# gallilmaimon/DISSC

Hardware: AMD Instinct MI355X
Metric: audio-sec/sec (RTF) HiFi-GAN resynth, 10s x32 batch (higher is better)
Workload: dtype f32

## Files before the change

dissc_amd/csrc/common.h:

```cpp
#pragma once
#include <hip/hip_runtime.h>
#include <stdint.h>
#include <stdio.h>

#include <atomic>
#include <mutex>
#include <string>
#include <vector>

#include "../../include/dissc_hip.h"

#ifndef DISSC_EXPERIMENTAL
#define DISSC_EXPERIMENTAL 0
#endif

namespace dissc {

void set_error(const char* fmt, ...);

#define DISSC_OPTION_LIST_DEFAULT(X) \
  X(multistream, 1, "multistream") \
  X(pair_dma, 1, "pair_dma") \
  X(precision, 0, "precision") \
  X(enc_precision, 0, "enc_precision") \
  X(use_mfma32, 1, "mfma32") \
  X(ragged_enum, 1, "ragged_enum") \
  X(lin128, 1, "lin128") \
  X(conv2s128, 1, "conv2s128") \
  X(xcd_order, 11, "xcd_order") \
  X(xcd_mg, 0, "xcd_mg") \
  X(small_grid, 1, "small_grid") \
  X(kernel_dbg, 0, "kernel_dbg") \
  X(wino_sv, 1, "wino_sv") \
  X(wino8_c64_wide, 3, "wino8_c64_wide") \
  X(wino8_mask, 0450770550, "wino8_mask") \
  X(wino8_r4_mask, 0770770010, "wino8_r4_mask") \
  X(wino8_r4, 1, "wino8_r4") \
  X(wino8, 1, "wino8") \
  X(wino, 1, "wino") \
  X(hubert_split, 1, "hubert_split") \
  X(pair_max_c, 32, "pair_max_c") \
  X(pair_f23, 3, "pair_f23") \
  X(pair_tc6, 3, "pair_tc6") \
  X(pair_f23_c64, 1, "pair_f23_c64")
#define DISSC_OPTION_LIST_EXPERIMENTAL(X) \
  X(graphs, 0, "graphs") \
  X(graph_frames, 2048, "graph_frames") \
  X(enc_tc, 0, "enc_tc") \
  X(s2tc_xmode, 0, "s2tc_xmode") \
  X(pair_wino, 0, "pair_wino") \
  X(pairw_chv, 2, "pairw_chv")
#if DISSC_EXPERIMENTAL
#define DISSC_OPTION_LIST(X) DISSC_OPTION_LIST_DEFAULT(X) DISSC_OPTION_LIST_EXPERIMENTAL(X)
#else
#define DISSC_OPTION_LIST(X) DISSC_OPTION_LIST_DEFAULT(X)
#endif
struct Options {
#define DISSC_OPT_FIELD(f, d, k) int f = d;
  DISSC_OPTION_LIST(DISSC_OPT_FIELD)
#undef DISSC_OPT_FIELD
#if !DISSC_EXPERIMENTAL
#define DISSC_OPT_CONST(f, d, k) static constexpr int f = d;
  DISSC_OPTION_LIST_EXPERIMENTAL(DISSC_OPT_CONST)
#undef DISSC_OPT_CONST
#endif
  int cfg_for_bm[5] = {6, 5, 7, 1, 0};
  int cfg32_for_bm[4] = {3, 2, 1, 0};
};
extern Options g_defaults;
extern thread_local const Options* t_opts;
inline const Options& opts() { return t_opts ? *t_opts : g_defaults; }
struct OptScope {
  const Options* prev;
  explicit OptScope(const Options* o) : prev(t_opts) { t_opts = o; }
  ~OptScope() { t_opts = prev; }
  OptScope(const OptScope&) = delete;
  OptScope& operator=(const OptScope&) = delete;
};

#define DISSC_HIP_CHECK(expr)                                                       \
  do {                                                                              \
    hipError_t _e = (expr);                                                         \
    if (_e != hipSuccess) {                                                         \
      dissc::set_error("%s failed: %s (%s:%d)", #expr, hipGetErrorString(_e),       \
                       __FILE__, __LINE__);                                         \
      return DISSC_EHIP;                                                            \
    }                                                                               \
  } while (0)

typedef float f32x4 __attribute__((ext_vector_type(4)));

struct DeviceOnce {
  std::mutex mu;
  std::atomic<bool> done[64];
  DeviceOnce() {
    for (auto& d : done) d.store(false, std::memory_order_relaxed);
  }
// ... 262 lines not shown
```

dissc_amd/csrc/generator.hip:

```cpp
#include <stdarg.h>
#include <stdlib.h>
#include <string.h>

#include <atomic>
#include <exception>
#include <functional>
#include <map>
#include <mutex>
#include <string>
#include <thread>
#include <tuple>
#include <vector>

#include <algorithm>

#include "common.h"

namespace dissc {

static thread_local char g_err[512] = "";
void set_error(const char* fmt, ...) {
  va_list ap;
  va_start(ap, fmt);
  vsnprintf(g_err, sizeof(g_err), fmt, ap);
// ... 2 lines not shown

Options g_defaults;
thread_local const Options* t_opts = nullptr;

}

using namespace dissc;

[[maybe_unused]] static int g_graph_hits = 0, g_graph_captures = 0;

enum class ChainForm : uint8_t {
  pairs,
  bf3_block,
  bf3_pairs,
};
enum class PairForm : uint8_t {
  direct,
  direct_dma,
  td,
  fused,
  fused_td,
};
enum class ConvForm : uint8_t { direct, f43, f63, f54 };
struct PairPlan {
  PairForm form = PairForm::direct;
  ConvForm conv[2] = {ConvForm::direct, ConvForm::direct};
  uint8_t reg_form = 0;
};
struct ChainPlan {
  ChainForm form = ChainForm::pairs;
  PairPlan pair[3];
};

constexpr int WINO_MIN_C = 64;
constexpr int WINO_C64_KMIN = 3;
static bool wino_wanted(int C, int KS) {
  if (!opts().wino || C < WINO_MIN_C) return false;
  if (C < 128 && KS < WINO_C64_KMIN) return false;
  return wino_supported(C, C, KS, 1);
}

static int w8_shape_bit(int C, int KS, int dil) {
  const int cls = C >= 256 ? 2 : C >= 128 ? 1 : 0;
  return 9 * cls + 3 * (KS == 11 ? 2 : KS == 7 ? 1 : 0) + (dil == 1 ? 0 : dil == 3 ? 1 : 2);
}
static ConvForm td_conv_form(int C, int KS, int dil) {
  if (!opts().wino8 || !wino8_supported(C, C, KS, dil) || !((opts().wino8_mask >> w8_shape_bit(C, KS, dil)) & 1))
    return ConvForm::f43;
  const bool r4 = opts().wino8_r4 && wino8_r4_supported(C, KS, dil) && ((opts().wino8_r4_mask >> w8_shape_bit(C, KS, dil)) & 1);
  return r4 ? ConvForm::f54 : ConvForm::f63;
}

static int pair_reg_form(int C, int KS, int dil) {
  if (C == 64) return KS == 3 && opts().pair_f23 != 0 && opts().pair_f23_c64 && pair_f23_supported(C, KS, dil) ? 1 : 0;
  if (C != 16 && C != 32) return 0;
  const int stage = C == 32 ? 1 : 2;
  if (KS == 3) return pair_f23_supported(C, KS, dil) && (opts().pair_f23 & (stage << 2)) ? 1 : 0;
  if (!(opts().pair_f23 & stage)) return 0;
  const int tc6_bit = (C == 32 ? 1 : 4) << (KS == 11 ? 1 : 0);
  if ((KS == 7 || KS == 11) && (opts().pair_tc6 & tc6_bit) && pair_tc6_supported(C, KS, dil)) return 2;
  return pair_f23_supported(C, KS, dil) ? 1 : 0;
}
static bool pairw_wanted(int C, int KS, int dil) {
  if (pair_reg_form(C, KS, dil)) return true;
  if (!opts().pair_wino || !pairw_supported(C, KS, dil)) return false;
  if (opts().pair_wino >= 2) return true;
  if (C == 32) return KS == 11 && dil <= 3;
  return C == 64 && KS == 3 && dil == 1;
}

static ChainPlan plan_chain(int C, int KS, const int* dil, int prec) {
  ChainPlan cp;
  if (prec == 1 && resblock_bf3_supported(C, KS, dil)) {
    cp.form = C >= 64 ? ChainForm::bf3_pairs : ChainForm::bf3_block;
    return cp;
  }
  bool fused = prec == 0 && (C < 32 || opts().use_mfma32) && C <= opts().pair_max_c;
  for (int m = 0; m < 3; ++m) fused = fused && respair_supported(C, KS, dil[m]);
  bool all_td = prec == 0 && opts().wino && C > 32 && wino_wanted(C, KS);
  for (int m = 0; m < 3; ++m) all_td = all_td && wino_supported(C, C, KS, dil[m]) && pairw_wanted(C, KS, dil[m]);
  for (int m = 0; m < 3; ++m) {
    PairPlan& p = cp.pair[m];
    const int d = dil[m];
    const bool td = prec == 0 && wino_wanted(C, KS) && wino_supported(C, C, KS, d);
    const bool fuse_td = prec == 0 && opts().wino && pairw_wanted(C, KS, d) && (C > 32 ? td : C <= opts().pair_max_c) &&
                         (fused || all_td || m == 0);
    if (fuse_td) {
      p.form = PairForm::fused_td;
      p.reg_form = (uint8_t)pair_reg_form(C, KS, d);
    } else if (fused) {
      p.form = PairForm::fused;
    } else if (td) {
      p.form = PairForm::td;
      p.conv[0] = td_conv_form(C, KS, d);
      p.conv[1] = td_conv_form(C, KS, 1);
    } else if (opts().pair_dma && prec == 0 && opts().use_mfma32 && C >= 32 && C % KC == 0) {
      p.form = PairForm::direct_dma;
    }
  }
  return cp;
}

static double pair_macs(const PairPlan& p, int C, int KS, bool executed) {
  const double direct = (double)C * C * KS;
  auto conv = [&](ConvForm f) {
    return f == ConvForm::f43 ? wino_executed_macs_per_t(C, KS)
         : f == ConvForm::f63 ? wino8_executed_macs_per_t(C, KS, 3)
// ... 567 lines not shown
  launch_conv_post(ACC, g->post_w, g->post_b, lengths, mul, B, ch, g->post_KS, Tmax * mul, ld,
                   (long long)ch * ld, 0.01f, wav_out, Tmax * mul, stream);
  DISSC_HIP_CHECK(hipGetLastError());
  return DISSC_OK;
}

int dissc_wav_postprocess(float* wav, const int32_t* n_samples, int B, int ld, void* stream) {
  if (!wav || !n_samples || B <= 0) {
    set_error("dissc_wav_postprocess: bad argument");
    return DISSC_EINVAL;
  }
  launch_wav_postprocess(wav, n_samples, B, ld, (hipStream_t)stream);
  DISSC_HIP_CHECK(hipGetLastError());
  return DISSC_OK;
}

static int conv_once(DevConv& dc, const float* x, float* y, const int32_t* lengths, int B,
                     int ldx, int ldo, int Lmax, float in_slope, hipStream_t stream) {
  int rc = run_conv(dc, x, y, nullptr, nullptr, lengths, Lmax, 1, B, dc.CIN, ldx, ldo, Lmax,
                    in_slope, EPI_STORE, 1.f, stream);
  hipError_t e = hipStreamSynchronize(stream);
  free_conv(dc);
  if (rc) return rc;
  DISSC_HIP_CHECK(e);
  return DISSC_OK;
}

int dissc_conv1d(const float* x, const float* w_host, const float* bias_host, float* y,
                 const int32_t* lengths, int B, int Cin, int Cout, int k, int dilation, int ldx,
                 int ldo, int Lmax, float in_slope, void* stream) {
  if (!x || !w_host || !y || k % 2 != 1 || dilation < 1) {
    set_error("dissc_conv1d: bad argument");
    return DISSC_EINVAL;
  }
  DevConv dc;
  int rc;
  if (opts().wino8 >= 2 && wino8_supported(Cout, Cin, k, dilation))
    rc = make_wino8(w_host, bias_host, Cout, k, dilation, dc, opts().wino8_r4 >= 2 && wino8_r4_supported(Cout, k, dilation) ? 4 : 3);
  else if (opts().wino >= 2 && wino_supported(Cout, Cin, k, dilation))
    rc = make_wino(w_host, bias_host, Cout, k, dilation, dc);
  else
    rc = make_conv(w_host, bias_host, Cout, Cin, k, dilation, dc);
  if (rc) return rc;
  return conv_once(dc, x, y, lengths, B, ldx, ldo, Lmax, in_slope, (hipStream_t)stream);
}

static int pair_run(int mode, const DevConv& c1, const DevConv& c2, const DevPairW& pw, const float* x, float* tmp, float* y,
                    float* acc, const int32_t* lengths, int B, int C, int ld, int Lmax, float slope, int epi, float mrf_div,
                    hipStream_t st) {
  int rc;
  switch (mode) {
    case 0:
    case 2:
      if ((rc = run_conv(c1, x, tmp, nullptr, nullptr, lengths, Lmax, 1, B, C, ld, ld, Lmax, slope, EPI_STORE, 1.f, st))) return rc;
      return run_conv(c2, tmp, y, x, acc, lengths, Lmax, 1, B, C, ld, ld, Lmax, slope, epi, mrf_div, st);
    case 1:
      return launch_respair(c1, c2, x, y, acc, lengths, Lmax, 1, B, Lmax, ld, slope, epi, mrf_div, st);
    case 3:
      return launch_respair_wino(pw, x, y, acc, lengths, Lmax, 1, B, Lmax, ld, slope, epi, mrf_div, st);
    default:
      set_error("pair mode %d", mode);
      return DISSC_EINVAL;
  }
}

static int pair_make(int mode, const float* w1, const float* b1, const float* w2, const float* b2, int C, int k, int d,
                     DevConv& c1, DevConv& c2, DevPairW& pw) {
  int rc;
  if (mode == 2) {
    if (!wino_supported(C, C, k, d) && !(C == 32 && (k == 3 || k == 7 || k == 11) && (d == 1 || d == 3 || d == 5))) {
      set_error("pair mode 2: no conv_wino instance for C = %d, k = %d, d = %d", C, k, d);
      return DISSC_EINVAL;
    }
    if ((rc = make_wino(w1, b1, C, k, d, c1))) return rc;
    return make_wino(w2, b2, C, k, 1, c2);
  }
  if (mode == 3) return make_pairw(w1, b1, w2, b2, C, k, d, pair_reg_form(C, k, d), pw);
  if ((rc = make_conv(w1, b1, C, C, k, d, c1))) return rc;
  return make_conv(w2, b2, C, C, k, 1, c2);
}

int dissc_respair1d(const float* x, const float* w1_host, const float* b1_host, const float* w2_host, const float* b2_host,
                    float* y, float* acc, const int32_t* lengths, int B, int C, int k, int dilation, int ld, int Lmax,
                    float slope, int epi, float mrf_div, int mode, void* stream) {
  if (!x || !w1_host || !w2_host || !y || k % 2 != 1 || dilation < 1 || B <= 0 || epi < EPI_RES || epi > EPI_MRF_DIV ||
      (epi != EPI_RES && !acc)) {
    set_error("dissc_respair1d: bad argument");
    return DISSC_EINVAL;
  }
  DevConv c1, c2;
  DevPairW pw;
  float* tmp = nullptr;
  int rc = pair_make(mode, w1_host, b1_host, w2_host, b2_host, C, k, dilation, c1, c2, pw);
  if (!rc && (mode == 0 || mode == 2) && hipMalloc((void**)&tmp, (size_t)B * C * ld * sizeof(float)) != hipSuccess) {
    set_error("dissc_respair1d: hipMalloc");
    rc = DISSC_ENOMEM;
  }
  if (!rc) rc = pair_run(mode, c1, c2, pw, x, tmp, y, acc, lengths, B, C, ld, Lmax, slope, epi, mrf_div, (hipStream_t)stream);
  const hipError_t e = hipStreamSynchronize((hipStream_t)stream);
  if (tmp) (void)hipFree(tmp);
  free_conv(c1);
  free_conv(c2);
  free_pairw(pw);
  if (rc) return rc;
  DISSC_HIP_CHECK(e);
  return DISSC_OK;
}

int dissc_pair_info(int C, int k, int dilation, int* form_out, int* tile_out) {
  const int form = pair_reg_form(C, k, dilation);
  if (!pair_form_supported(form, C, k, dilation)) {
    set_error("dissc_pair_info: no instance for C = %d, k = %d, dilation %d", C, k, dilation);
    return DISSC_EINVAL;
  }
  if (form_out) *form_out = form;
  if (tile_out) *tile_out = pair_reg_tile(form, C, k, dilation);
  return DISSC_OK;
}

int dissc_conv_info(int Cin, int Cout, int k, int dilation, int up, int B, int Lmax_out, DisscConvLaunch* out, int max_out,
                    int* n_out) {
  if (Cin < 1 || Cout < 1 || k < 1 || dilation < 1 || up < 1 || B < 1 || Lmax_out < 1 || max_out < 0 || (max_out && !out) ||
      (up == 1 && k % 2 != 1) || (up > 1 && ((k - up) % 2 != 0 || k < up || dilation != 1))) {
    set_error("dissc_conv_info: bad argument");
    return DISSC_EINVAL;
  }
  std::vector<ConvTGroup> plan;
  if (up > 1) convT_groups(Cout, k, up, plan);
  else plan.push_back(ConvTGroup{0, 1, 0, k});
  int n = 0;
  for (const ConvTGroup& g : plan) {
    DevConv dc;
    conv_geometry(dc, Cout * g.np, Cin, g.ntap, up > 1 ? 1 : dilation, 1, 1, up > 1 ? -g.dlo : -1);
    int family, cfg, bm, bn;
    const int rc = conv_launch_info(dc, B, Lmax_out, &family, &cfg, &bm, &bn);
    if (rc) return rc;
    if (n < max_out) {
      DisscConvLaunch& o = out[n];
      o.family = family; o.cfg = cfg; o.bm = bm; o.bn = bn; o.rows = dc.M;
      o.p0 = g.p0; o.np = g.np; o.ntap = g.ntap;
      o.pad_left = dc.pad_left >= 0 ? dc.pad_left : ((dc.KS - 1) * dc.dil) / 2;
    }
    ++n;
  }
  if (n_out) *n_out = n;
  return DISSC_OK;
}
// ... 187 lines not shown
```

dissc_amd/csrc/pair_host.hip:

```cpp
#include <string.h>

#include <algorithm>
#include <vector>

#include "common.h"
#include "respair_f23.h"

namespace dissc {

bool pair_f23_supported(int C, int KS, int dil) {
  if (!(dil == 1 || dil == 3 || dil == 5)) return false;
  if (C == 64) return KS == 3;
  return (C == 16 || C == 32) && (KS == 11 || (KS == 3 && DISSC_EXPERIMENTAL));
}
bool pair_tc6_supported(int C, int KS, int dil) { return C == 32 && (KS == 7 || KS == 11) && (dil == 1 || dil == 3 || dil == 5); }
bool pairw_supported(int C, int KS, int dil) {
  if (!pairw43_built()) return false;
  if (!(dil == 1 || dil == 3 || dil == 5)) return false;
  if (C == 32) return KS == 7 || KS == 11;
  if (C == 64) return KS == 3;
  return false;
}
bool pair_form_supported(int form, int C, int KS, int dil) {
  return form == 2 ? pair_tc6_supported(C, KS, dil) : form == 1 ? pair_f23_supported(C, KS, dil) : pairw_supported(C, KS, dil);
}

static const double kF23G[4][3] = {{1.0, 0.0, 0.0}, {0.5, 0.5, 0.5}, {0.5, -0.5, 0.5}, {0.0, 0.0, 1.0}};
static const double kTc6G[6][4] = {{1.0 / 4, 0.0, 0.0, 0.0},
                                   {-1.0 / 6, -1.0 / 6, -1.0 / 6, -1.0 / 6},
                                   {-1.0 / 6, 1.0 / 6, -1.0 / 6, 1.0 / 6},
                                   {1.0 / 24, 2.0 / 24, 4.0 / 24, 8.0 / 24},
                                   {1.0 / 24, -2.0 / 24, 4.0 / 24, -8.0 / 24},
                                   {0.0, 0.0, 0.0, 1.0}};

static std::vector<float> transform_taps(const float* w, int C, int KS, const double* G, int points, int taps) {
  const int NS = (KS + taps - 1) / taps;
  std::vector<float> U((size_t)points * C * C * NS);
  size_t o = 0;
  for (int p = 0; p < points; ++p)
    for (int cc = 0; cc < C * C; ++cc)
      for (int j = 0; j < NS; ++j) {
        double u = 0.0;
        for (int i = 0; i < taps; ++i)
          if (j + NS * i < KS) u += G[p * taps + i] * (double)w[(size_t)cc * KS + j + NS * i];
        U[o++] = (float)u;
      }
  return U;
}

static int pack_pair_reg(const float* w, float** dev, int C, int KS, int form) {
  if ((form != 1 && form != 2) || (C != 16 && C != 32 && C != 64) || (form == 2 && C != 32) || (C == 64 && KS != 3)) {
    set_error("pack_pair_reg: no layout for form %d, C = %d", form, C);
    return DISSC_EINVAL;
  }
  const int points = form == 2 ? 6 : 4, taps = form == 2 ? 4 : 3, NS = (KS + taps - 1) / taps;
  const std::vector<float> U = transform_taps(w, C, KS, form == 2 ? &kTc6G[0][0] : &kF23G[0][0], points, taps);
  auto u = [&](int p, int co, int ci, int j) { return U[(((size_t)p * C + co) * C + ci) * NS + j]; };
  std::vector<float> packed(U.size());
  size_t o = 0;
  if (C == 16) {
    for (int j = 0; j < NS; ++j)
      for (int p = 0; p < 4; ++p)
        for (int lane = 0; lane < 64; ++lane)
          for (int cq = 0; cq < 4; ++cq) packed[o++] = u(p, lane & 15, 4 * cq + (lane >> 4), j);
  } else if (C == 64) {
    for (int st = 0; st < 8; ++st)
      for (int p = 0; p < 4; ++p)
        for (int mi = 0; mi < 2; ++mi)
          for (int lane = 0; lane < 64; ++lane)
            for (int e = 0; e < 4; ++e) packed[o++] = u(p, 32 * mi + (lane & 31), 8 * st + 2 * e + (lane >> 5), 0);
  } else if (form == 1) {
    for (int c = 0; c < 2; ++c)
      for (int j = 0; j < NS; ++j)
        for (int p = 0; p < 4; ++p)
          for (int hf = 0; hf < 2; ++hf)
            for (int lane = 0; lane < 64; ++lane)
              for (int e = 0; e < 4; ++e) packed[o++] = u(p, lane & 31, 16 * c + 2 * (4 * hf + e) + (lane >> 5), j);
  } else {
    for (int c = 0; c < 2; ++c)
      for (int j = 0; j < NS; ++j)
        for (int hf = 0; hf < 2; ++hf)
          for (int p = 0; p < 6; ++p)
            for (int lane = 0; lane < 64; ++lane)
              for (int e = 0; e < 4; ++e) packed[o++] = u(p, lane & 31, 16 * c + 2 * (4 * hf + e) + (lane >> 5), j);
  }
  return upload(packed, dev);
}

int make_pairw(const float* w1, const float* b1, const float* w2, const float* b2, int C, int KS, int dil, int form, DevPairW& pw) {
  pw.form = form;
  if (!pair_form_supported(form, C, KS, dil)) {
    set_error("make_pairw: no instance for C = %d, k = %d, dilation %d", C, KS, dil);
    return DISSC_EINVAL;
  }
  pw.C = C; pw.KS = KS; pw.dil = dil;
  auto pack = [&](const float* w, float** dev) {
    return form ? pack_pair_reg(w, dev, C, KS, form) : pack_pairw43(w, C, KS, dev);
  };
  int rc = pack(w1, &pw.w1);
  if (!rc) rc = pack(w2, &pw.w2);
  std::vector<float> bb(C, 0.f);
  if (b1) memcpy(bb.data(), b1, C * sizeof(float));
  if (!rc) rc = upload(bb, &pw.b1);
  std::fill(bb.begin(), bb.end(), 0.f);
  if (b2) memcpy(bb.data(), b2, C * sizeof(float));
  if (!rc) rc = upload(bb, &pw.b2);
  return rc;
}

void free_pairw(DevPairW& pw) {
  for (float** q : {&pw.w1, &pw.w2, &pw.b1, &pw.b2}) {
    if (*q) (void)hipFree(*q);
    *q = nullptr;
  }
}

template <auto Kernel, class Geo>
static int launch_pair_reg(const PairArgs& a, int B, int Lmax, hipStream_t stream, bool want_max_lds) {
  static DeviceOnce attr_once;
  if (want_max_lds) DISSC_HIP_CHECK(attr_once.max_lds(reinterpret_cast<const void*>(Kernel), 160 * 1024));
  dim3 grid((Lmax + Geo::WOUT - 1) / Geo::WOUT, B);
  hipLaunchKernelGGL(Kernel, grid, dim3(256), sizeof(float) * Geo::C * Geo::XW, stream, a);
  DISSC_HIP_CHECK(hipGetLastError());
  return DISSC_OK;
}

#define DISSC_TC6(K_, D_) DISSC_CASE(2, 32, respair32_tc6_kernel, Tc6Geo, true, K_, D_)
#define DISSC_F23_32(K_, D_) DISSC_CASE(1, 32, respair32_f23_kernel, F23Geo32, true, K_, D_)
#define DISSC_F23_16(K_, D_) DISSC_CASE(1, 16, respair16_f23_kernel, F23Geo16, false, K_, D_)
#define DISSC_F23_64(K_, D_) DISSC_CASE(1, 64, respair64_f23_kernel, F23Geo64, true, K_, D_)
#define DISSC_PAIR_REG_INSTANCES                                                                          \
  DISSC_PAIR_TC6_SHAPES(DISSC_TC6) DISSC_PAIR_F23_SHAPES(DISSC_F23_32) DISSC_PAIR_F23_SHAPES(DISSC_F23_16) \
  DISSC_PAIR_F23_C64_SHAPES(DISSC_F23_64)

int pair_reg_tile(int form, int C, int KS, int dil) {
#define DISSC_CASE(FORM_, C_, KERNEL_, GEO_, MAX_LDS_, K_, D_) \
  if (form == FORM_ && C == C_ && KS == K_ && dil == D_) return GEO_<K_, D_>::WOUT;
  DISSC_PAIR_REG_INSTANCES
#undef DISSC_CASE
  return 0;
}

static int launch_pair_f23(const DevPairW& pw, const float* x, float* out, float* acc, const int32_t* lengths, int len_default,
                           int len_mul, int B, int Lmax, int ld, float slope, int epi, float mrf_div, hipStream_t stream) {
  PairArgs a;
  a.x = x; a.out = out; a.acc = acc; a.w1 = pw.w1; a.w2 = pw.w2; a.b1 = pw.b1; a.b2 = pw.b2;
  a.lengths = lengths; a.len_default = len_default; a.len_mul = len_mul; a.ld = ld;
  a.bstride = (long long)pw.C * ld; a.slope = slope; a.mrf_div = mrf_div; a.epi = epi; a.dbg = opts().kernel_dbg;
#define DISSC_CASE(FORM_, C_, KERNEL_, GEO_, MAX_LDS_, K_, D_)       \
  if (pw.form == FORM_ && pw.C == C_ && pw.KS == K_ && pw.dil == D_) \
    return launch_pair_reg<KERNEL_<K_, D_>, GEO_<K_, D_>>(a, B, Lmax, stream, MAX_LDS_);
  DISSC_PAIR_REG_INSTANCES
#undef DISSC_CASE
  set_error("launch_pair_f23: no instance of form %d for C = %d, k = %d, dilation %d", pw.form, pw.C, pw.KS, pw.dil);
  return DISSC_EINVAL;
}

int launch_respair_wino(const DevPairW& pw, const float* x, float* out, float* acc, const int32_t* lengths, int len_default,
                        int len_mul, int B, int Lmax, int ld, float slope, int epi, float mrf_div, hipStream_t stream) {
  if (!pw.w1 || epi == EPI_STORE || x == out || ld < 4 || ld % 4 || misaligned16(x) || misaligned16(out) || misaligned16(acc) ||
      B <= 0 || Lmax <= 0) {
    set_error("launch_respair_wino: bad argument (C=%d k=%d d=%d ld=%d epi=%d)", pw.C, pw.KS, pw.dil, ld, epi);
    return DISSC_EINVAL;
  }
  if (pw.form) return launch_pair_f23(pw, x, out, acc, lengths, len_default, len_mul, B, Lmax, ld, slope, epi, mrf_div, stream);
  if (pairw43_built())
    return launch_pairw43(pw, x, out, acc, lengths, len_default, len_mul, B, Lmax, ld, slope, epi, mrf_div, stream);
  set_error("launch_respair_wino: no instance (the F(4,3) pair kernel is only in DISSC_EXPERIMENTAL=1 builds)");
  return DISSC_EINVAL;
}

}
```

dissc_amd/csrc/respair_f23.h:

```cpp
#pragma once
#include "common.h"
#include "ragged_epi.h"

namespace dissc {

struct PairArgs {
  const float* x;
  float* out;
  float* acc;
  const float* w1;
  const float* w2;
  const float* b1;
  const float* b2;
  const int32_t* lengths;
  int len_default, len_mul;
  int ld;
  long long bstride;
  float slope, mrf_div;
  int epi;
  int dbg;
};

template <int WOUT>
__device__ __forceinline__ bool pair_tile(const PairArgs& a, int B, int& b, int& len, int& o0) {
// ... 31 lines not shown
      if (i >= C * NV) continue;
      const int r = i / NV, v = i - r * NV;
      const int t = tb + 4 * v;
      f32x4 val = sv[it];
#pragma unroll
      for (int e = 0; e < 4; ++e) val[e] = ((t + e) >= 0 && (t + e) < len) ? (val[e] > 0.f ? val[e] : val[e] * slope) : 0.f;
      *reinterpret_cast<f32x4*>(xs + r * XW + 4 * v) = val;
    }
  }
}

template <int C, int XW, int W1, int NT>
__device__ __forceinline__ void pair_zero_beyond_t(float* xs, int tid) {
  for (int i = tid; i < C * (XW - W1); i += NT) {
    const int r = i / (XW - W1), v = i - r * (XW - W1);
    xs[r * XW + W1 + v] = 0.f;
  }
}

template <class AccOld>
__device__ __forceinline__ void pair_store_tail(const PairArgs& a, int epi, size_t idx, f32x4 v, float bz, const f32x4& rv,
                                                AccOld acc_old, int elo, int ehi) {
  if (elo == 0 && ehi == 4) {
#pragma unroll
    for (int e = 0; e < 4; ++e) v[e] = (v[e] + bz) + rv[e];
    epi_store_res(epi, quad_at(a.out + idx), quad_at(a.acc + idx), v, acc_old, a.mrf_div);
  } else {
    for (int e = elo; e < ehi; ++e)
      epi_store_res(epi, a.out + idx + e, a.acc + idx + e, (v[e] + bz) + a.x[idx + e], [&] { return a.acc[idx + e]; }, a.mrf_div);
  }
}

template <int C_, int PROWS, int KS_, int DIL, int WCOLS = 64>
struct F23Geo {
  static constexpr int KS = KS_, NS = (KS_ + 2) / 3, C = C_, NW = 4;
  static constexpr int P2 = (KS - 1) / 2, P1 = P2 * DIL;
  static constexpr int D1 = DIL * NS, D2 = NS;
  static constexpr int NCOLS = WCOLS * NW;
  static constexpr int NU1 = NCOLS / D1, NC1 = NU1 * D1, W1 = 2 * NC1;
  static constexpr int NU2 = NCOLS / D2, NC2 = NU2 * D2, W2 = 2 * NC2;
  static constexpr int WOUT = ((W1 - 2 * P2) < W2 ? (W1 - 2 * P2) : W2) & ~3;
  static constexpr int REACH1 = (3 * NS - 1) * DIL, REACH2 = 3 * NS - 1;
  static constexpr int XW1 = round32_16(3 + W1 + REACH1);
  static constexpr int XW2 = round32_16(W2 + REACH2 + 1);
  static constexpr int XW = XW1 > XW2 ? XW1 : XW2;
  static constexpr int PW = 2 * WCOLS + 4;
  static_assert(NW * PROWS * PW <= C * XW, "the epilogue patches fit the buffer");
  static_assert(W1 <= XW && W2 + REACH2 < XW, "T fits the buffer");
};
template <int KS, int DIL> using F23Geo32 = F23Geo<32, 8, KS, DIL>;
template <int KS, int DIL> using F23Geo16 = F23Geo<16, 16, KS, DIL>;
template <int KS, int DIL> using F23Geo64 = F23Geo<64, 8, KS, DIL, 32>;

template <int KS_, int DIL>
struct Tc6Geo {
  static constexpr int KS = KS_, NS = (KS_ + 3) / 4, C = 32, NW = 4;
  static constexpr int P2 = (KS - 1) / 2, P1 = P2 * DIL;
  static constexpr int D1 = DIL * NS, D2 = NS;
  static constexpr int NCOLS = 32 * NW;
  static constexpr int NU1 = NCOLS / D1, NC1 = NU1 * D1, W1 = 3 * NC1;
  static constexpr int NCW2 = 32 / D2 * D2, OW = 3 * NCW2, W2 = NW * OW;
  static constexpr int WOUT = ((W1 - 2 * P2) < W2 ? (W1 - 2 * P2) : W2) & ~3;
  static constexpr int REACH1 = (4 * NS - 1) * DIL, REACH2 = 4 * NS - 1;
  static constexpr int XW1 = (3 + W1 + REACH1 + 3) & ~3;
  static constexpr int XW2 = (W2 + REACH2 + 3) & ~3;
  static constexpr int XW = XW1 > XW2 ? XW1 : XW2;
  static constexpr int PW = 96 + 4;
  static constexpr int OCC = 3 * 4 * C * XW <= 160 * 1024 ? 3 : 2;
  static_assert(3 + OW <= PW - 1 && NW * 8 * PW <= C * XW, "the epilogue patches fit the buffer");
  static_assert(W1 <= XW && WOUT + 2 * P2 <= W1 && WOUT <= W2, "T fits the buffer and covers what the owned outputs read");
};

template <int KS, int DIL> __global__ void respair32_f23_kernel(const PairArgs a);
template <int KS, int DIL> __global__ void respair32_tc6_kernel(const PairArgs a);
template <int KS, int DIL> __global__ void respair16_f23_kernel(const PairArgs a);
template <int KS, int DIL> __global__ void respair64_f23_kernel(const PairArgs a);
#if DISSC_EXPERIMENTAL
#define DISSC_PAIR_F23_SHAPES(X) X(11, 1) X(11, 3) X(11, 5) X(3, 1) X(3, 3) X(3, 5)
#else
#define DISSC_PAIR_F23_SHAPES(X) X(11, 1) X(11, 3) X(11, 5)
#endif
#define DISSC_PAIR_F23_C64_SHAPES(X) X(3, 1) X(3, 3) X(3, 5)
#define DISSC_PAIR_TC6_SHAPES(X) X(7, 1) X(7, 3) X(7, 5) X(11, 1) X(11, 3) X(11, 5)

}
```

dissc_amd/csrc/respair_f23.hip:

```cpp
#include "common.h"
#include "respair_f23.h"

namespace dissc {

template <int KS_, int DIL>
__global__ void __launch_bounds__(256, 2) respair32_f23_kernel(const PairArgs a) {
  using G = F23Geo32<KS_, DIL>;
  constexpr int C = G::C, NW = G::NW, NT = 64 * NW, NS = G::NS, P2 = G::P2, P1 = G::P1, D1 = G::D1, D2 = G::D2, XW = G::XW,
                W1 = G::W1, NC1 = G::NC1, NC2 = G::NC2, WOUT = G::WOUT, PW = G::PW;
  extern __shared__ __attribute__((aligned(16))) float xs[];

  int b, len, o0;
  if (!pair_tile<WOUT>(a, gridDim.y, b, len, o0)) return;
  const int tid = threadIdx.x, lane = tid & 63, wave = tid >> 6;
  const int l31 = lane & 31, h = lane >> 5;
  const int tin0 = o0 - P2 - P1;
  const int tb = tin0 & ~3, sh = tin0 - tb;
  const float slope = a.slope;
  const float* xb = a.x + (size_t)b * a.bstride;

  pair_stage_window<C, XW, NT>(a, xb, xs, tb, len, tid);

  int base1[2], base2[2];
#pragma unroll
// ... 92 lines not shown
  clear();
  if (!(a.dbg & 1)) taps(a.w2, xs, base2, 0, 1, D2);

  __syncthreads();
  float* ep = xs + wave * (8 * PW);
  const int prow = lane >> 5, pc4 = lane & 31;
  const int ncol = wave * 128 + 4 * pc4;
  const int tcol = o0 + ncol;
  const size_t ob = (size_t)b * a.bstride;
  const bool live = ncol < WOUT && tcol < len;
  const int epi = a.epi;
  const bool rmw = epi != EPI_RES && epi != EPI_MRF_SET;
  if (a.dbg & 4) {
    if (acc[0][0][0] == 123.f) a.out[0] = 1.f;
    return;
  }
#pragma unroll
  for (int qd = 0; qd < 4; ++qd) {
    f32x4 rv[4], pa[4];
#pragma unroll
    for (int p = 0; p < 4; ++p) {
      const int row = 8 * qd + 2 * p + prow;
      const int tc = tcol > a.ld - 4 ? a.ld - 4 : tcol;
      rv[p] = *reinterpret_cast<const f32x4*>(a.x + ob + (size_t)row * a.ld + tc);
      if (rmw && live && tcol + 4 <= len) pa[p] = *reinterpret_cast<const f32x4*>(a.acc + ob + (size_t)row * a.ld + tcol);
    }
    __builtin_amdgcn_wave_barrier();
#pragma unroll
    for (int ni = 0; ni < 2; ++ni) {
      const int cl = ni * 32 + l31;
      const int pe = 2 * D2 * (cl / D2) + (cl % D2);
#pragma unroll
      for (int r = 0; r < 4; ++r) {
        const int rr = 4 * qd + r;
        const float y0 = acc[0][ni][rr], y1 = acc[1][ni][rr], y2 = acc[2][ni][rr], y3 = acc[3][ni][rr];
        ep[(r + 4 * h) * PW + pe] = (y0 + y1) + y2;
        ep[(r + 4 * h) * PW + pe + D2] = (y1 - y2) - y3;
      }
    }
    __builtin_amdgcn_wave_barrier();
#pragma unroll
    for (int p = 0; p < 4; ++p) {
      const int prw = 2 * p + prow;
      f32x4 v = *reinterpret_cast<const f32x4*>(ep + prw * PW + 4 * pc4);
      if (!live) continue;
      const int row = 8 * qd + prw;
      const float bz = a.b2[row];
      const size_t idx = ob + (size_t)row * a.ld + tcol;
      pair_store_tail(a, epi, idx, v, bz, rv[p], [&] { return pa[p]; }, 0, len - tcol < 4 ? len - tcol : 4);
    }
  }
}

template <int KS_, int DIL>
__global__ void __launch_bounds__(256, (Tc6Geo<KS_, DIL>::OCC)) respair32_tc6_kernel(const PairArgs a) {
  using G = Tc6Geo<KS_, DIL>;
  constexpr int C = G::C, NW = G::NW, NT = 64 * NW, NS = G::NS, P2 = G::P2, P1 = G::P1, D1 = G::D1, D2 = G::D2, XW = G::XW,
                W1 = G::W1, NC1 = G::NC1, NCW2 = G::NCW2, OW = G::OW, WOUT = G::WOUT, PW = G::PW;
  extern __shared__ __attribute__((aligned(16))) float xs[];

  int b, len, o0;
  if (!pair_tile<WOUT>(a, gridDim.y, b, len, o0)) return;
  const int tid = threadIdx.x, lane = tid & 63, wave = tid >> 6;
  const int l31 = lane & 31, h = lane >> 5;
  const int tin0 = o0 - P2 - P1;
  const int tb = tin0 & ~3, sh = tin0 - tb;
  const float slope = a.slope;
  const float* xb = a.x + (size_t)b * a.bstride;

  pair_stage_window<C, XW, NT>(a, xb, xs, tb, len, tid);

  int base1, base2;
  {
    const int c = wave * 32 + l31;
    const int c1 = c < NC1 ? c : NC1 - 1, c2 = l31 < NCW2 ? l31 : NCW2 - 1;
    base1 = 3 * D1 * (c1 / D1) + (c1 % D1);
    base2 = wave * OW + 3 * D2 * (c2 / D2) + (c2 % D2);
  }
  typedef float f32x16f __attribute__((ext_vector_type(16)));
  f32x16f acc[6];
  auto clear = [&]() __attribute__((always_inline)) {
#pragma unroll
    for (int p = 0; p < 6; ++p)
#pragma unroll
      for (int e = 0; e < 16; ++e) acc[p][e] = 0.f;
  };
  auto taps = [&](const float* wq, const float* src, int base, int dstep, int dunit) __attribute__((always_inline)) {
    const __amdgpu_buffer_rsrc_t wr = wave_rsrc(wq, 0x7ffffff0u);
    const unsigned lane16 = lane * 16u;
    constexpr int NST = 2 * NS * 2;
    const unsigned wstep = (a.dbg & 8) ? 0u : 6 * 1024u;
    f32x4 av[6], avn[6];
#pragma unroll
    for (int p = 0; p < 6; ++p) av[p] = rsrc_load16(wr, lane16, p * 1024u);
#pragma unroll
    for (int st = 0; st < NST; ++st) {
      const int sn = st + 1 < NST ? st + 1 : st;
#pragma unroll
      for (int p = 0; p < 6; ++p) avn[p] = rsrc_load16(wr, lane16, sn * wstep + p * 1024u);
      __builtin_amdgcn_sched_barrier(0);
      const int chunk = (st >> 1) / NS, j = (st >> 1) % NS, hf = st & 1;
#pragma unroll
      for (int e = 0; e < 4; ++e) {
        const int row = 16 * chunk + 2 * (4 * hf + e) + h;
        const float* q = src + row * XW + base + j * dstep;
        const float x0 = q[0], x1 = q[dunit], x2 = q[2 * dunit], x3 = q[3 * dunit], x4 = q[4 * dunit], x5 = q[5 * dunit];
        const float pe = __builtin_fmaf(-4.f, x2, x4), po = __builtin_fmaf(-4.f, x1, x3), re = x4 - x2, ro = x3 - x1;
        float bq[6];
        bq[0] = __builtin_fmaf(4.f, x0, __builtin_fmaf(-5.f, x2, x4));
        bq[1] = pe + po;
        bq[2] = pe - po;
        bq[3] = __builtin_fmaf(2.f, ro, re);
        bq[4] = __builtin_fmaf(-2.f, ro, re);
        bq[5] = __builtin_fmaf(4.f, x1, __builtin_fmaf(-5.f, x3, x5));
#pragma unroll
        for (int p = 0; p < 6; ++p) acc[p] = __builtin_amdgcn_mfma_f32_32x32x2f32(av[p][e], bq[p], acc[p], 0, 0, 0);
      }
      __builtin_amdgcn_sched_barrier(0);
#pragma unroll
      for (int p = 0; p < 6; ++p) av[p] = avn[p];
    }
  };
  auto outs = [&](int r, float& y0, float& y1, float& y2) __attribute__((always_inline)) {
    const float s12 = acc[1][r] + acc[2][r], d12 = acc[1][r] - acc[2][r];
    const float s34 = acc[3][r] + acc[4][r], d34 = acc[3][r] - acc[4][r];
    y0 = (acc[0][r] + s12) + s34;
    y1 = __builtin_fmaf(2.f, d34, d12);
    y2 = __builtin_fmaf(4.f, s34, s12) + acc[5][r];
  };

  __syncthreads();
  clear();
  if (!(a.dbg & 1)) taps(a.w1, xs + sh, base1, DIL, D1);

  __syncthreads();
  pair_zero_beyond_t<C, XW, W1, NT>(xs, tid);
  {
    const int c = wave * 32 + l31;
    if (c < NC1 && !(a.dbg & 2)) {
      const int p0 = 3 * D1 * (c / D1) + (c % D1);
      const int t0 = o0 - P2 + p0;
      const bool in0 = t0 >= 0 && t0 < len, in1 = t0 + D1 >= 0 && t0 + D1 < len, in2 = t0 + 2 * D1 >= 0 && t0 + 2 * D1 < len;
#pragma unroll
      for (int r = 0; r < 16; ++r) {
        const int row = (r & 3) + 8 * (r >> 2) + 4 * h;
        const float bz = a.b1[row];
        float v0, v1, v2;
        outs(r, v0, v1, v2);
        v0 += bz; v1 += bz; v2 += bz;
        v0 = v0 > 0.f ? v0 : v0 * slope;
        v1 = v1 > 0.f ? v1 : v1 * slope;
        v2 = v2 > 0.f ? v2 : v2 * slope;
        xs[row * XW + p0] = in0 ? v0 : 0.f;
        xs[row * XW + p0 + D1] = in1 ? v1 : 0.f;
        xs[row * XW + p0 + 2 * D1] = in2 ? v2 : 0.f;
      }
    }
  }
  __syncthreads();
  clear();
  if (!(a.dbg & 1)) taps(a.w2, xs, base2, 1, D2);

  __syncthreads();
  float* ep = xs + wave * (8 * PW);
  const int prow = lane >> 5, pc4 = lane & 31;
  const int ws = wave * OW, woff = ws & 3;
  const int ncol = ws - woff + 4 * pc4;
  const int tcol = o0 + ncol;
  const size_t ob = (size_t)b * a.bstride;
  const int wend = ws + OW < WOUT ? ws + OW : WOUT;
  const int elo = ncol < ws ? ws - ncol : 0;
  const int ehi = (wend - ncol < len - tcol ? wend - ncol : len - tcol) < 4 ? (wend - ncol < len - tcol ? wend - ncol : len - tcol) : 4;
  const bool live = ehi > elo;
  const int epi = a.epi;
  const bool rmw = epi != EPI_RES && epi != EPI_MRF_SET;
  if (a.dbg & 4) {
    if (acc[0][0] == 123.f) a.out[0] = 1.f;
    return;
  }
  const int cl = l31 < NCW2 ? l31 : NCW2 - 1;
  const int pcol = woff + 3 * D2 * (cl / D2) + (cl % D2);
#pragma unroll
  for (int qd = 0; qd < 4; ++qd) {
    __builtin_amdgcn_sched_barrier(0);
    f32x4 rv[4], pa[4];
    const int tc = tcol > a.ld - 4 ? a.ld - 4 : tcol;
#pragma unroll
    for (int p = 0; p < 4; ++p) rv[p] = *reinterpret_cast<const f32x4*>(a.x + ob + (size_t)(8 * qd + 2 * p + prow) * a.ld + tc);
    if (rmw) {
#pragma unroll
      for (int p = 0; p < 4; ++p) pa[p] = *reinterpret_cast<const f32x4*>(a.acc + ob + (size_t)(8 * qd + 2 * p + prow) * a.ld + tc);
    }
    __builtin_amdgcn_wave_barrier();
#pragma unroll
    for (int r = 0; r < 4; ++r) {
      float y0, y1, y2;
      outs(4 * qd + r, y0, y1, y2);
      ep[(r + 4 * h) * PW + pcol] = y0;
      ep[(r + 4 * h) * PW + pcol + D2] = y1;
      ep[(r + 4 * h) * PW + pcol + 2 * D2] = y2;
    }
    __builtin_amdgcn_wave_barrier();
#pragma unroll
    for (int p = 0; p < 4; ++p) {
      const int prw = 2 * p + prow;
      f32x4 v = *reinterpret_cast<const f32x4*>(ep + prw * PW + (4 * pc4 < PW - 4 ? 4 * pc4 : PW - 4));
      if (!live) continue;
      const int row = 8 * qd + prw;
      const float bz = a.b2[row];
      const size_t idx = ob + (size_t)row * a.ld + tcol;
      pair_store_tail(a, epi, idx, v, bz, rv[p], [&] { return pa[p]; }, elo, ehi);
    }
  }
}

template <int KS_, int DIL>
__global__ void __launch_bounds__(256, 2) respair64_f23_kernel(const PairArgs a) {
  using G = F23Geo64<KS_, DIL>;
  constexpr int C = G::C, NW = G::NW, NT = 64 * NW, P2 = G::P2, P1 = G::P1, D1 = G::D1, D2 = G::D2, XW = G::XW, W1 = G::W1,
                NC1 = G::NC1, NC2 = G::NC2, WOUT = G::WOUT, PW = G::PW;
  static_assert(G::NS == 1 && D2 == 1 && XW % 2 == 0, "one sub-filter; conv_1's samples pair up into 8-byte reads");
  extern __shared__ __attribute__((aligned(16))) float xs[];

  int b, len, o0;
  if (!pair_tile<WOUT>(a, gridDim.y, b, len, o0)) return;
  const int tid = threadIdx.x, lane = tid & 63, wave = tid >> 6;
  const int l31 = lane & 31, h = lane >> 5;
  const int tin0 = o0 - P2 - P1;
  const int tb = tin0 & ~3, sh = tin0 - tb;
  const float slope = a.slope;
  const float* xb = a.x + (size_t)b * a.bstride;

  pair_stage_window<C, XW, NT, 2>(a, xb, xs, tb, len, tid);

  const int col = wave * 32 + l31;
  const int c1 = col < NC1 ? col : NC1 - 1, c2 = col < NC2 ? col : NC2 - 1;
  const int base1 = 2 * D1 * (c1 / D1) + (c1 % D1), base2 = 2 * D2 * (c2 / D2) + (c2 % D2);
  typedef float f32x16f __attribute__((ext_vector_type(16)));
  typedef float f32x2f __attribute__((ext_vector_type(2)));
  f32x16f acc[4][2];
  auto clear = [&]() __attribute__((always_inline)) {
#pragma unroll
    for (int p = 0; p < 4; ++p)
#pragma unroll
      for (int mi = 0; mi < 2; ++mi)
#pragma unroll
        for (int e = 0; e < 16; ++e) acc[p][mi][e] = 0.f;
  };
  auto taps = [&](const float* wq, const float* src, int dunit) __attribute__((always_inline)) {
    const __amdgpu_buffer_rsrc_t wr = wave_rsrc(wq, 0x7ffffff0u);
    const unsigned lane16 = lane * 16u;
    constexpr int NST = C / 8;
    f32x4 av[4][2], avn[4][2];
#pragma unroll
    for (int p = 0; p < 4; ++p)
#pragma unroll
      for (int mi = 0; mi < 2; ++mi) av[p][mi] = rsrc_load16(wr, lane16, (p * 2 + mi) * 1024u);
#pragma unroll
    for (int st = 0; st < NST; ++st) {
      const int sn = st + 1 < NST ? st + 1 : st;
#pragma unroll
      for (int p = 0; p < 4; ++p)
#pragma unroll
        for (int mi = 0; mi < 2; ++mi) avn[p][mi] = rsrc_load16(wr, lane16, ((sn * 4 + p) * 2 + mi) * 1024u);
      __builtin_amdgcn_sched_barrier(0);
#pragma unroll
// ... 62 lines not shown
  const bool live = ncol < WOUT && tcol < len;
  const int epi = a.epi;
  const bool rmw = epi != EPI_RES && epi != EPI_MRF_SET;
  if (a.dbg & 4) {
    if (acc[0][0][0] == 123.f) a.out[0] = 1.f;
    return;
  }
  const int pcol = 2 * l31;
#pragma unroll
  for (int mq = 0; mq < 8; ++mq) {
    const int mi = mq >> 2, qd = mq & 3;
    __builtin_amdgcn_sched_barrier(0);
    f32x4 rv[2], pa[2];
    const int tc = tcol > a.ld - 4 ? a.ld - 4 : tcol;
#pragma unroll
    for (int p = 0; p < 2; ++p) {
      const int row = 8 * mq + 4 * p + prow;
      rv[p] = *reinterpret_cast<const f32x4*>(a.x + ob + (size_t)row * a.ld + tc);
      if (rmw && live && tcol + 4 <= len) pa[p] = *reinterpret_cast<const f32x4*>(a.acc + ob + (size_t)row * a.ld + tcol);
    }
    __builtin_amdgcn_wave_barrier();
#pragma unroll
    for (int r = 0; r < 4; ++r) {
      const int rr = 4 * qd + r;
      const float y0 = acc[0][mi][rr], y1 = acc[1][mi][rr], y2 = acc[2][mi][rr], y3 = acc[3][mi][rr];
      f32x2f v;
      v[0] = (y0 + y1) + y2;
      v[1] = (y1 - y2) - y3;
      *reinterpret_cast<f32x2f*>(ep + (r + 4 * h) * PW + pcol) = v;
    }
    __builtin_amdgcn_wave_barrier();
#pragma unroll
    for (int p = 0; p < 2; ++p) {
      const int prw = 4 * p + prow;
      f32x4 v = *reinterpret_cast<const f32x4*>(ep + prw * PW + 4 * pc4);
      if (!live) continue;
      const int row = 8 * mq + prw;
      const float bz = a.b2[row];
      const size_t idx = ob + (size_t)row * a.ld + tcol;
      pair_store_tail(a, epi, idx, v, bz, rv[p], [&] { return pa[p]; }, 0, len - tcol < 4 ? len - tcol : 4);
    }
  }
}

#define DISSC_INSTANCE(K_, D_) template __global__ void respair32_f23_kernel<K_, D_>(const PairArgs);
DISSC_PAIR_F23_SHAPES(DISSC_INSTANCE)
#undef DISSC_INSTANCE
#define DISSC_INSTANCE(K_, D_) template __global__ void respair32_tc6_kernel<K_, D_>(const PairArgs);
DISSC_PAIR_TC6_SHAPES(DISSC_INSTANCE)
#undef DISSC_INSTANCE
#define DISSC_INSTANCE(K_, D_) template __global__ void respair64_f23_kernel<K_, D_>(const PairArgs);
DISSC_PAIR_F23_C64_SHAPES(DISSC_INSTANCE)
#undef DISSC_INSTANCE

}
```

Baseline: 10020.

## Extend fused tc6 residual-pair kernel to 64-channel k=7 blocks

```diff
diff --git a/dissc_amd/csrc/common.h b/dissc_amd/csrc/common.h
--- a/dissc_amd/csrc/common.h
+++ b/dissc_amd/csrc/common.h
@@ -42,7 +42,8 @@
   X(pair_max_c, 32, "pair_max_c") \
   X(pair_f23, 3, "pair_f23") \
   X(pair_tc6, 3, "pair_tc6") \
-  X(pair_f23_c64, 1, "pair_f23_c64")
+  X(pair_f23_c64, 1, "pair_f23_c64") \
+  X(pair_tc6_c64, 1, "pair_tc6_c64")
 #define DISSC_OPTION_LIST_EXPERIMENTAL(X) \
   X(graphs, 0, "graphs") \
   X(graph_frames, 2048, "graph_frames") \
diff --git a/dissc_amd/csrc/generator.hip b/dissc_amd/csrc/generator.hip
--- a/dissc_amd/csrc/generator.hip
+++ b/dissc_amd/csrc/generator.hip
@@ -78,7 +78,12 @@
 }
 
 static int pair_reg_form(int C, int KS, int dil) {
-  if (C == 64) return KS == 3 && opts().pair_f23 != 0 && opts().pair_f23_c64 && pair_f23_supported(C, KS, dil) ? 1 : 0;
+  if (C == 64) {
+    if (opts().pair_f23 == 0) return 0;
+    if (KS == 3) return opts().pair_f23_c64 && pair_f23_supported(C, KS, dil) ? 1 : 0;
+    const int bit = KS == 7 ? 1 : KS == 11 ? 2 : 0;
+    return (opts().pair_tc6_c64 & bit) && pair_tc6_supported(C, KS, dil) ? 2 : 0;
+  }
   if (C != 16 && C != 32) return 0;
   const int stage = C == 32 ? 1 : 2;
   if (KS == 3) return pair_f23_supported(C, KS, dil) && (opts().pair_f23 & (stage << 2)) ? 1 : 0;
@@ -752,6 +757,7 @@
   switch (mode) {
     case 0:
     case 2:
+    case 4:
       if ((rc = run_conv(c1, x, tmp, nullptr, nullptr, lengths, Lmax, 1, B, C, ld, ld, Lmax, slope, EPI_STORE, 1.f, st))) return rc;
       return run_conv(c2, tmp, y, x, acc, lengths, Lmax, 1, B, C, ld, ld, Lmax, slope, epi, mrf_div, st);
     case 1:
@@ -776,6 +782,14 @@
     return make_wino(w2, b2, C, k, 1, c2);
   }
   if (mode == 3) return make_pairw(w1, b1, w2, b2, C, k, d, pair_reg_form(C, k, d), pw);
+  if (mode == 4) {
+    if (!wino_supported(C, C, k, d) || !wino_supported(C, C, k, 1)) {
+      set_error("pair mode 4: no transform-domain conv instance for C = %d, k = %d, d = %d", C, k, d);
+      return DISSC_EINVAL;
+    }
+    if ((rc = make_pair_conv(td_conv_form(C, k, d), w1, b1, C, k, d, c1))) return rc;
+    return make_pair_conv(td_conv_form(C, k, 1), w2, b2, C, k, 1, c2);
+  }
   if ((rc = make_conv(w1, b1, C, C, k, d, c1))) return rc;
   return make_conv(w2, b2, C, C, k, 1, c2);
 }
@@ -792,7 +806,7 @@
   DevPairW pw;
   float* tmp = nullptr;
   int rc = pair_make(mode, w1_host, b1_host, w2_host, b2_host, C, k, dilation, c1, c2, pw);
-  if (!rc && (mode == 0 || mode == 2) && hipMalloc((void**)&tmp, (size_t)B * C * ld * sizeof(float)) != hipSuccess) {
+  if (!rc && (mode == 0 || mode == 2 || mode == 4) && hipMalloc((void**)&tmp, (size_t)B * C * ld * sizeof(float)) != hipSuccess) {
     set_error("dissc_respair1d: hipMalloc");
     rc = DISSC_ENOMEM;
   }
diff --git a/dissc_amd/csrc/pair_host.hip b/dissc_amd/csrc/pair_host.hip
--- a/dissc_amd/csrc/pair_host.hip
+++ b/dissc_amd/csrc/pair_host.hip
@@ -13,7 +13,7 @@
   if (C == 64) return KS == 3;
   return (C == 16 || C == 32) && (KS == 11 || (KS == 3 && DISSC_EXPERIMENTAL));
 }
-bool pair_tc6_supported(int C, int KS, int dil) { return C == 32 && (KS == 7 || KS == 11) && (dil == 1 || dil == 3 || dil == 5); }
+bool pair_tc6_supported(int C, int KS, int dil) { return (C == 32 || C == 64) && (KS == 7 || KS == 11) && (dil == 1 || dil == 3 || dil == 5); }
 bool pairw_supported(int C, int KS, int dil) {
   if (!pairw43_built()) return false;
   if (!(dil == 1 || dil == 3 || dil == 5)) return false;
@@ -49,7 +49,7 @@
 }
 
 static int pack_pair_reg(const float* w, float** dev, int C, int KS, int form) {
-  if ((form != 1 && form != 2) || (C != 16 && C != 32 && C != 64) || (form == 2 && C != 32) || (C == 64 && KS != 3)) {
+  if ((form != 1 && form != 2) || (C != 16 && C != 32 && C != 64) || (form == 2 && C == 16) || (form == 1 && C == 64 && KS != 3)) {
     set_error("pack_pair_reg: no layout for form %d, C = %d", form, C);
     return DISSC_EINVAL;
   }
@@ -63,6 +63,14 @@
       for (int p = 0; p < 4; ++p)
         for (int lane = 0; lane < 64; ++lane)
           for (int cq = 0; cq < 4; ++cq) packed[o++] = u(p, lane & 15, 4 * cq + (lane >> 4), j);
+  } else if (C == 64 && form == 2) {
+    for (int mi = 0; mi < 2; ++mi)
+      for (int c = 0; c < 4; ++c)
+        for (int j = 0; j < NS; ++j)
+          for (int hf = 0; hf < 2; ++hf)
+            for (int p = 0; p < 6; ++p)
+              for (int lane = 0; lane < 64; ++lane)
+                for (int e = 0; e < 4; ++e) packed[o++] = u(p, 32 * mi + (lane & 31), 16 * c + 2 * (4 * hf + e) + (lane >> 5), j);
   } else if (C == 64) {
     for (int st = 0; st < 8; ++st)
       for (int p = 0; p < 4; ++p)
@@ -126,12 +134,13 @@
 }
 
 #define DISSC_TC6(K_, D_) DISSC_CASE(2, 32, respair32_tc6_kernel, Tc6Geo, true, K_, D_)
+#define DISSC_TC6_64(K_, D_) DISSC_CASE(2, 64, respair64_tc6_kernel, Tc6Geo64, false, K_, D_)
 #define DISSC_F23_32(K_, D_) DISSC_CASE(1, 32, respair32_f23_kernel, F23Geo32, true, K_, D_)
 #define DISSC_F23_16(K_, D_) DISSC_CASE(1, 16, respair16_f23_kernel, F23Geo16, false, K_, D_)
 #define DISSC_F23_64(K_, D_) DISSC_CASE(1, 64, respair64_f23_kernel, F23Geo64, true, K_, D_)
 #define DISSC_PAIR_REG_INSTANCES                                                                          \
   DISSC_PAIR_TC6_SHAPES(DISSC_TC6) DISSC_PAIR_F23_SHAPES(DISSC_F23_32) DISSC_PAIR_F23_SHAPES(DISSC_F23_16) \
-  DISSC_PAIR_F23_C64_SHAPES(DISSC_F23_64)
+  DISSC_PAIR_F23_C64_SHAPES(DISSC_F23_64) DISSC_PAIR_TC6_SHAPES(DISSC_TC6_64)
 
 int pair_reg_tile(int form, int C, int KS, int dil) {
 #define DISSC_CASE(FORM_, C_, KERNEL_, GEO_, MAX_LDS_, K_, D_) \
diff --git a/dissc_amd/csrc/respair_f23.h b/dissc_amd/csrc/respair_f23.h
--- a/dissc_amd/csrc/respair_f23.h
+++ b/dissc_amd/csrc/respair_f23.h
@@ -107,14 +107,14 @@
 template <int KS, int DIL> using F23Geo16 = F23Geo<16, 16, KS, DIL>;
 template <int KS, int DIL> using F23Geo64 = F23Geo<64, 8, KS, DIL, 32>;
 
-template <int KS_, int DIL>
-struct Tc6Geo {
-  static constexpr int KS = KS_, NS = (KS_ + 3) / 4, C = 32, NW = 4;
+template <int C_, int KS_, int DIL_>
+struct Tc6GeoC {
+  static constexpr int KS = KS_, DIL = DIL_, NS = (KS_ + 3) / 4, C = C_, NW = 4, RB = C_ / 32, NCT = NW / RB;
   static constexpr int P2 = (KS - 1) / 2, P1 = P2 * DIL;
   static constexpr int D1 = DIL * NS, D2 = NS;
-  static constexpr int NCOLS = 32 * NW;
+  static constexpr int NCOLS = 32 * NCT;
   static constexpr int NU1 = NCOLS / D1, NC1 = NU1 * D1, W1 = 3 * NC1;
-  static constexpr int NCW2 = 32 / D2 * D2, OW = 3 * NCW2, W2 = NW * OW;
+  static constexpr int NCW2 = 32 / D2 * D2, OW = 3 * NCW2, W2 = NCT * OW;
   static constexpr int WOUT = ((W1 - 2 * P2) < W2 ? (W1 - 2 * P2) : W2) & ~3;
   static constexpr int REACH1 = (4 * NS - 1) * DIL, REACH2 = 4 * NS - 1;
   static constexpr int XW1 = (3 + W1 + REACH1 + 3) & ~3;
@@ -122,14 +122,18 @@
   static constexpr int XW = XW1 > XW2 ? XW1 : XW2;
   static constexpr int PW = 96 + 4;
   static constexpr int OCC = 3 * 4 * C * XW <= 160 * 1024 ? 3 : 2;
+  static_assert(C == 32 || C == 64, "one or two 32-row blocks");
   static_assert(3 + OW <= PW - 1 && NW * 8 * PW <= C * XW, "the epilogue patches fit the buffer");
   static_assert(W1 <= XW && WOUT + 2 * P2 <= W1 && WOUT <= W2, "T fits the buffer and covers what the owned outputs read");
 };
+template <int KS, int DIL> using Tc6Geo = Tc6GeoC<32, KS, DIL>;
+template <int KS, int DIL> using Tc6Geo64 = Tc6GeoC<64, KS, DIL>;
 
 template <int KS, int DIL> __global__ void respair32_f23_kernel(const PairArgs a);
 template <int KS, int DIL> __global__ void respair32_tc6_kernel(const PairArgs a);
 template <int KS, int DIL> __global__ void respair16_f23_kernel(const PairArgs a);
 template <int KS, int DIL> __global__ void respair64_f23_kernel(const PairArgs a);
+template <int KS, int DIL> __global__ void respair64_tc6_kernel(const PairArgs a);
 #if DISSC_EXPERIMENTAL
 #define DISSC_PAIR_F23_SHAPES(X) X(11, 1) X(11, 3) X(11, 5) X(3, 1) X(3, 3) X(3, 5)
 #else
diff --git a/dissc_amd/csrc/respair_f23.hip b/dissc_amd/csrc/respair_f23.hip
--- a/dissc_amd/csrc/respair_f23.hip
+++ b/dissc_amd/csrc/respair_f23.hip
@@ -168,30 +168,30 @@
   }
 }
 
-template <int KS_, int DIL>
-__global__ void __launch_bounds__(256, (Tc6Geo<KS_, DIL>::OCC)) respair32_tc6_kernel(const PairArgs a) {
-  using G = Tc6Geo<KS_, DIL>;
+template <class G>
+__device__ __forceinline__ void pair_tc6_body(const PairArgs a) {
   constexpr int C = G::C, NW = G::NW, NT = 64 * NW, NS = G::NS, P2 = G::P2, P1 = G::P1, D1 = G::D1, D2 = G::D2, XW = G::XW,
-                W1 = G::W1, NC1 = G::NC1, NCW2 = G::NCW2, OW = G::OW, WOUT = G::WOUT, PW = G::PW;
+                W1 = G::W1, NC1 = G::NC1, NCW2 = G::NCW2, OW = G::OW, WOUT = G::WOUT, PW = G::PW, RB = G::RB, DIL = G::DIL;
   extern __shared__ __attribute__((aligned(16))) float xs[];
 
   int b, len, o0;
   if (!pair_tile<WOUT>(a, gridDim.y, b, len, o0)) return;
   const int tid = threadIdx.x, lane = tid & 63, wave = tid >> 6;
   const int l31 = lane & 31, h = lane >> 5;
+  const int ct = wave / RB, mrow = 32 * (wave % RB);
   const int tin0 = o0 - P2 - P1;
   const int tb = tin0 & ~3, sh = tin0 - tb;
   const float slope = a.slope;
   const float* xb = a.x + (size_t)b * a.bstride;
 
-  pair_stage_window<C, XW, NT>(a, xb, xs, tb, len, tid);
+  pair_stage_window<C, XW, NT, RB>(a, xb, xs, tb, len, tid);
 
   int base1, base2;
   {
-    const int c = wave * 32 + l31;
+    const int c = ct * 32 + l31;
     const int c1 = c < NC1 ? c : NC1 - 1, c2 = l31 < NCW2 ? l31 : NCW2 - 1;
     base1 = 3 * D1 * (c1 / D1) + (c1 % D1);
-    base2 = wave * OW + 3 * D2 * (c2 / D2) + (c2 % D2);
+    base2 = ct * OW + 3 * D2 * (c2 / D2) + (c2 % D2);
   }
   typedef float f32x16f __attribute__((ext_vector_type(16)));
   f32x16f acc[6];
@@ -204,7 +204,7 @@
   auto taps = [&](const float* wq, const float* src, int base, int dstep, int dunit) __attribute__((always_inline)) {
     const __amdgpu_buffer_rsrc_t wr = wave_rsrc(wq, 0x7ffffff0u);
     const unsigned lane16 = lane * 16u;
-    constexpr int NST = 2 * NS * 2;
+    constexpr int NST = C / 16 * NS * 2;
     const unsigned wstep = (a.dbg & 8) ? 0u : 6 * 1024u;
     f32x4 av[6], avn[6];
 #pragma unroll
@@ -245,21 +245,22 @@
     y2 = __builtin_fmaf(4.f, s34, s12) + acc[5][r];
   };
 
+  const int wslab = (wave % RB) * (C / 16 * NS * 2 * 6 * 256);
   __syncthreads();
   clear();
-  if (!(a.dbg & 1)) taps(a.w1, xs + sh, base1, DIL, D1);
+  if (!(a.dbg & 1)) taps(a.w1 + wslab, xs + sh, base1, DIL, D1);
 
   __syncthreads();
   pair_zero_beyond_t<C, XW, W1, NT>(xs, tid);
   {
-    const int c = wave * 32 + l31;
+    const int c = ct * 32 + l31;
     if (c < NC1 && !(a.dbg & 2)) {
       const int p0 = 3 * D1 * (c / D1) + (c % D1);
       const int t0 = o0 - P2 + p0;
       const bool in0 = t0 >= 0 && t0 < len, in1 = t0 + D1 >= 0 && t0 + D1 < len, in2 = t0 + 2 * D1 >= 0 && t0 + 2 * D1 < len;
 #pragma unroll
       for (int r = 0; r < 16; ++r) {
-        const int row = (r & 3) + 8 * (r >> 2) + 4 * h;
+        const int row = mrow + (r & 3) + 8 * (r >> 2) + 4 * h;
         const float bz = a.b1[row];
         float v0, v1, v2;
         outs(r, v0, v1, v2);
@@ -275,12 +276,12 @@
   }
   __syncthreads();
   clear();
-  if (!(a.dbg & 1)) taps(a.w2, xs, base2, 1, D2);
+  if (!(a.dbg & 1)) taps(a.w2 + wslab, xs, base2, 1, D2);
 
   __syncthreads();
   float* ep = xs + wave * (8 * PW);
   const int prow = lane >> 5, pc4 = lane & 31;
-  const int ws = wave * OW, woff = ws & 3;
+  const int ws = ct * OW, woff = ws & 3;
   const int ncol = ws - woff + 4 * pc4;
   const int tcol = o0 + ncol;
   const size_t ob = (size_t)b * a.bstride;
@@ -302,10 +303,10 @@
     f32x4 rv[4], pa[4];
     const int tc = tcol > a.ld - 4 ? a.ld - 4 : tcol;
 #pragma unroll
-    for (int p = 0; p < 4; ++p) rv[p] = *reinterpret_cast<const f32x4*>(a.x + ob + (size_t)(8 * qd + 2 * p + prow) * a.ld + tc);
+    for (int p = 0; p < 4; ++p) rv[p] = *reinterpret_cast<const f32x4*>(a.x + ob + (size_t)(mrow + 8 * qd + 2 * p + prow) * a.ld + tc);
     if (rmw) {
 #pragma unroll
-      for (int p = 0; p < 4; ++p) pa[p] = *reinterpret_cast<const f32x4*>(a.acc + ob + (size_t)(8 * qd + 2 * p + prow) * a.ld + tc);
+      for (int p = 0; p < 4; ++p) pa[p] = *reinterpret_cast<const f32x4*>(a.acc + ob + (size_t)(mrow + 8 * qd + 2 * p + prow) * a.ld + tc);
     }
     __builtin_amdgcn_wave_barrier();
 #pragma unroll
@@ -322,12 +323,21 @@
       const int prw = 2 * p + prow;
       f32x4 v = *reinterpret_cast<const f32x4*>(ep + prw * PW + (4 * pc4 < PW - 4 ? 4 * pc4 : PW - 4));
       if (!live) continue;
-      const int row = 8 * qd + prw;
+      const int row = mrow + 8 * qd + prw;
       const float bz = a.b2[row];
       const size_t idx = ob + (size_t)row * a.ld + tcol;
       pair_store_tail(a, epi, idx, v, bz, rv[p], [&] { return pa[p]; }, elo, ehi);
     }
   }
+}
+
+template <int KS_, int DIL>
+__global__ void __launch_bounds__(256, (Tc6Geo<KS_, DIL>::OCC)) respair32_tc6_kernel(const PairArgs a) {
+  pair_tc6_body<Tc6Geo<KS_, DIL>>(a);
+}
+template <int KS_, int DIL>
+__global__ void __launch_bounds__(256, (Tc6Geo64<KS_, DIL>::OCC)) respair64_tc6_kernel(const PairArgs a) {
+  pair_tc6_body<Tc6Geo64<KS_, DIL>>(a);
 }
 
 template <int KS_, int DIL>
@@ -496,5 +506,8 @@
 #define DISSC_INSTANCE(K_, D_) template __global__ void respair64_f23_kernel<K_, D_>(const PairArgs);
 DISSC_PAIR_F23_C64_SHAPES(DISSC_INSTANCE)
 #undef DISSC_INSTANCE
+#define DISSC_INSTANCE(K_, D_) template __global__ void respair64_tc6_kernel<K_, D_>(const PairArgs);
+DISSC_PAIR_TC6_SHAPES(DISSC_INSTANCE)
+#undef DISSC_INSTANCE
 
 }
```

Result: faster. 10160, median of 6 (+1.4%).
